# v1o/flyimg

Measured on AMD Instinct MI355X. Metric: input Mpix/s resize+smartcrop at 1/2/4/8 MI355X; % of HBM roofline, higher is better.
Workload: dtype u8

## Files before the change

### flyimg_amd/csrc/fi_batch.cpp

```cpp
#include "fi_runtime.h"

using namespace fi;

static int launch_batch(fi_ctx *c, const Exec &E, const BatchPlan &Bp, const Packed &K, uint8_t *ab, uint8_t *wb,
                        Slot &S) {
  S.tail = c->sc_stream;
  S.ap_lo = S.ap_hi = 0;
  const int32_t *ai = (const int32_t *)c->heap_i.p;
  const float *af = (const float *)c->heap_f.p;
  const double *ad = (const double *)c->heap_d.p;
  const ScParamsDev PD = to_dev(E.params);
  auto desc_p = [&](const Launch &L) { return ab + L.desc_off; };
  auto pre_p = [&](const Launch &L) { return (const int32_t *)(ab + L.prefix_off); };
  Timer tb(c, "batch", 0, c->stream, c->sc_stream);
  {
    Timer t(c, "resize", Bp.resize_bytes);
    if (K.L0.tiles)
      hipLaunchKernelGGL(k_rs_copy, dim3(K.L0.tiles), dim3(256), 0, c->stream, (const ResizeDesc *)desc_p(K.L0),
                         pre_p(K.L0), K.L0.n);
    const bool fork = c->vr_fork && c->rs2_stream && Bp.vrl.size() >= 2;
    if (fork) {
      if (!c->rs_fork) HIP_TRY(hipEventCreateWithFlags(&c->rs_fork, hipEventDisableTiming));
      if (!c->rs_join) HIP_TRY(hipEventCreateWithFlags(&c->rs_join, hipEventDisableTiming));
      HIP_TRY(hipEventRecord(c->rs_fork, c->stream));
// ... 331 lines not shown
    if (rc != FI_OK && first == FI_OK) first = rc;
  }
  if (first != FI_OK) return first;
  return FI_OK;
}
static int wait_slot(fi_ctx *c, int slot) {
  int first = FI_OK;
  while (c->slots[slot].busy && !c->inflight.empty()) {
    const int rc = finalize_front(c);
    if (rc != FI_OK && first == FI_OK) first = rc;
  }
  return first;
}

extern "C" {

int fi_debug_host_plan(const fi_image *imgs, int32_t n, int32_t iters, double *ms) {
  static fi_ctx *c = nullptr;
  static std::vector<uint8_t> last_blob;
  static size_t last_work = 0;
  static double last[7] = {0, 0, 0, 0, 0, 0, 0};
  if (!imgs && n == 0) {
    if (c && getenv("FI_PLAN_PROF"))
      for (const auto &kv : c->stats) fprintf(stderr, "%s %.1f ms (%lld)\n", kv.first.c_str(), kv.second.ms, (long long)kv.second.launches);
    delete c;
    c = nullptr;
    std::vector<uint8_t>().swap(last_blob);
    return FI_OK;
  }
  if (!imgs && n == 1) {
    if (c) c->stats.clear();
    return FI_OK;
  }
  if (!imgs && n == 2) {
    if (!ms) return set_err(FI_EINVAL, "ms is NULL");
    ms[0] = ms[1] = ms[2] = 0;
    if (c) {
      ms[0] = (double)c->stats["plan_path_vr"].launches;
      ms[1] = (double)c->stats["plan_vertical_first"].launches;
      ms[2] = (double)c->stats["plan_vr_launches"].launches;
    }
    return FI_OK;
  }
  if (!imgs && n == 3) {
    if (!ms) return set_err(FI_EINVAL, "ms is NULL");
    uint64_t h = 1469598103934665603ull;
    for (uint8_t x : last_blob) h = (h ^ x) * 1099511628211ull;
    for (int k = 0; k < 8; k++) h = (h ^ (((uint64_t)last_work >> (8 * k)) & 255)) * 1099511628211ull;
    last[0] = (double)(uint32_t)h;
    last[1] = (double)(uint32_t)(h >> 32);
    for (int k = 0; k < 7; k++) ms[k] = last[k];
    return FI_OK;
  }
  if (!imgs || n <= 0 || iters <= 0 || !ms) return set_err(FI_EINVAL, "bad arguments");
  if (!c) {
    c = new fi_ctx();
    c->host_only = true;
    c->timing = true;
    if (const char *e = getenv("FI_VR_RS")) c->vr_rs = e[0] == '1';
  }
  std::vector<fi_image> v(imgs, imgs + n);
  uint8_t *wb = reinterpret_cast<uint8_t *>((uintptr_t)1 << 40);
  int rc = FI_OK;
  for (int it = 0; it < iters && rc == FI_OK; it++) {
    const double t0 = now_ms();
    Exec E;
    E.c = c;
    fi_smartcrop_default_params(&E.params);
    rc = heap_prepare(c, E);
    if (rc) break;
    BatchPlan Bp;
    PlanTimes T;
    Packed K;
    const double vr0 = c->stats["host_plan_vr"].ms;
    plan_batch(c, E, Bp, v.data(), n, T);
    place_batch(c, E, Bp, K, wb, T);
    int nvr = 0;
    for (const BatchPlan::VrLaunch &V : Bp.vrl) nvr += V.images;
    c->stats["plan_path_vr"].launches += nvr;
    c->stats["plan_vertical_first"].launches += (int64_t)Bp.vdescs.size() - nvr;
    c->stats["plan_vr_launches"].launches += (int64_t)Bp.vrl.size();
    last_blob.swap(E.blob.b);
    last[2] = (double)last_blob.size();
    last[3] = (double)Bp.vtiles.size();
    last[4] = (double)Bp.vrtiles.size();
    last[5] = (double)Bp.htiles.size();
    last[6] = (double)Bp.sitems.size();
    last_work = E.work.size;
    if (!heap_fits(c, E)) heap_reset(c);
    else {
      c->heap_i.used = (size_t)E.bi + (E.ai.size() + 15) / 16 * 16;
      c->heap_f.used = (size_t)E.bf + (E.af.size() + 15) / 16 * 16;
      c->heap_d.used = (size_t)E.bd + (E.ad.size() + 15) / 16 * 16;
    }
    ms[0] += T.images - t0;
    ms[1] += T.sc - T.images;
    ms[2] += T.workspace - T.sc;
    ms[3] += T.vm - T.workspace;
    ms[4] += c->stats["host_plan_vr"].ms - vr0;
    ms[5] += T.hv - T.vm;
    ms[6] += T.blob - T.hv;
  }
  return rc;
}

int fi_process_batch_device(fi_ctx *c, fi_image *imgs, int32_t n) {
// ... 154 lines not shown
```

### flyimg_amd/csrc/fi_internal.h

```cpp
#pragma once
#include <hip/hip_runtime.h>
#include <stdint.h>

#include "../../include/flyimg_hip.h"

namespace fi {

constexpr int kMaxChannels = 3;

struct DevAxis {
  int32_t n;
  int32_t start;
  int32_t count;
  int32_t woff;
  int32_t maxtaps;
  int32_t src_lo;
  int32_t src_hi;
  int32_t touched;
  int32_t wbase;
  int32_t wd;
};

struct ResizeDesc {
  const uint8_t *src;
// ... 53 lines not shown
  int32_t ybox_first, hrows;
  int32_t hb, hk, ksh;
  int32_t vb, vk, ksv;
  int32_t hkT;
  int32_t prep;
  int32_t hm;
  int32_t hm_rows, hm_ks, hm_pitch, hm_nb;
  int32_t hmB, hmC, hmS0;
  int32_t vq;
  int32_t fz;
  int32_t fd;
  int32_t vqA, vqC, vqK0;
  int32_t cx;
  int32_t cx_kv, cx_tp;
  int32_t cxA, cxK0;
  int32_t cx_pad;
  uint8_t *tbuf;
  uint8_t *red;
  uint8_t *hbuf;
  uint8_t *pre;
  uint32_t *maps;
  int32_t crop0, ncrops;
  int32_t score0;
  double prescale;
  double T[3];
  int32_t result;
  int32_t exact_all;
  int32_t sg0, ngrp;
  int32_t sg_lds, sg_pad;
};

constexpr int kPrepRows = 16;
constexpr int kVqRows = 14;
constexpr int kPrepMaxLds = 64 * 1024;
constexpr int kHxRb = 8;
constexpr int kFzMaxLds = 80 * 1024;
__host__ __device__ inline uint32_t sc_spread3(uint32_t x) {
  x = (x | (x << 8)) & 0x0000F00Fu;
  x = (x | (x << 4)) & 0x000C30C3u;
  return (x | (x << 2)) & 0x00249249u;
}
__host__ __device__ inline uint32_t sc_colour_key(uint32_t r, uint32_t g, uint32_t b) {
  return (sc_spread3(r) << 2) | (sc_spread3(g) << 1) | sc_spread3(b);
}
constexpr int kFdSlots = 3;
constexpr int kFdCWaves = 14;
constexpr int kFdMaxLds = 160 * 1024;
__host__ __device__ inline int fd_rp(int W) { return (W * 3 + 15) & ~15; }
__host__ __device__ inline int fd_slot_bytes(int W) { return (16 * fd_rp(W) + 1023) & ~1023; }
__host__ __device__ inline int fd_ring_off(int W, int PP) {
  const int tail = 3 * PP - fd_rp(W);
  return kFdSlots * fd_slot_bytes(W) + (tail > 0 ? (tail + 15) & ~15 : 0);
}
__host__ __device__ inline int fd_tab_off(int W, int PP, int aw) {
  const int apitch = (aw * 3 + 15) & ~15, lpitch = (aw + 3) & ~3;
  return fd_ring_off(W, PP) + 80 * apitch + 16 * apitch + 16 * lpitch;
}
__host__ __device__ inline int fd_lds(int W, int PP, int aw, int ah) {
  return fd_tab_off(W, PP, aw) + (ah + kVqRows - 1) / kVqRows * 3072 + 4 * ah;
}
constexpr int kScoreLdsMaps = 112 * 1024;
constexpr int kScoreMaxCrops = 1024;
constexpr int kSgSlots = 3;
constexpr int kSgDigits = 5;
constexpr int kSgPlanes = 7;
constexpr int kSgMax = 2;
constexpr int kSgMaxKs = 2;
constexpr int kSgMaxCrops = kSgMax * 16 * kSgSlots;
constexpr int kScore3Lds = 160 * 1024 - 4608;
__host__ __device__ inline int sg_pitch(int aw) { return (aw + 7) & ~7; }
struct ScGroup {
  int32_t bfrag;
  int32_t nrows, ks, ybase;
  int32_t nm, nslot, q, step;
  int32_t x0[16];
  int32_t S[kSgDigits];
  int32_t pad[3];
};

#ifndef FI_MFMA_I8_MAP
#define FI_MFMA_I8_MAP 1
#endif
__host__ __device__ inline int mfma_i8_k(int l, int j) {
#if FI_MFMA_I8_MAP == 1
  return 16 * (l >> 4) + j;
#else
  return j < 8 ? 8 * (l >> 4) + j : 32 + 8 * (l >> 4) + (j - 8);
#endif
}
struct MStrip {
  int32_t x0, x1, b0, nbytes;
  int32_t c_lo, ncols, pitch, nocb, ks;
  int32_t lut_px0, lut_n;
  int32_t frag, s0, lut;
  int32_t vpitch;
  int32_t frag2;
};
constexpr int kHmMaxLds = 64 * 1024;

struct VDesc {
  const uint8_t *src;
  int64_t src_stride;
  uint8_t *dst;
  int64_t dst_stride;
  int32_t ew, eh, rot, gray;
  int32_t rows, nrows, row0, rstep;
  int32_t plo, pn, pblk, plast;
  int32_t pmeta;
  int32_t frag;
// ... 169 lines not shown
```

### flyimg_amd/csrc/fi_sc_plan.cpp

```cpp
#include "fi_runtime.h"

using namespace fi;

ScParamsDev fi::to_dev(const fi_smartcrop_params &p) {
  ScParamsDev d{};
  d.detail_weight = p.detail_weight;
  d.edge_radius = p.edge_radius;
  d.edge_weight = p.edge_weight;
  d.outside_importance = p.outside_importance;
  d.saturation_bias = p.saturation_bias;
  d.saturation_brightness_max = p.saturation_brightness_max;
  d.saturation_brightness_min = p.saturation_brightness_min;
  d.saturation_threshold = p.saturation_threshold;
  d.saturation_weight = p.saturation_weight;
  d.skin_bias = p.skin_bias;
  d.skin_brightness_max = p.skin_brightness_max;
  d.skin_brightness_min = p.skin_brightness_min;
  for (int i = 0; i < 3; i++) d.skin_color[i] = p.skin_color[i];
  d.skin_threshold = p.skin_threshold;
  d.skin_weight = p.skin_weight;
  d.rule_of_thirds = p.rule_of_thirds;
  return d;
}
static uint64_t params_hash(const fi_smartcrop_params &p) {
// ... 367 lines not shown
    } else if ((int64_t)d.aw * d.ah * 4 <= kScoreLdsMaps) {
      sl.push_back(d);
      X->sl_px = std::max(X->sl_px, d.aw * d.ah);
    } else {
      sg.push_back(d);
    }
  }
  X->red = add_launch(B, SL.descs, sred, [](const ScDesc &d) { return d.rh; });
  X->hp = add_launch(B, SL.descs, shp, [](const ScDesc &d) { return d.hrows; });
  X->vp = add_launch(B, SL.descs, svp, [](const ScDesc &d) { return d.ah; });
  X->maps = add_launch(B, SL.descs, smaps, [](const ScDesc &d) { return d.ah; });
  X->hm_off = B.addv(hm);
  X->nhm = (int)hm.size();
  X->vq_off = B.addv(vq);
  X->vm_off = B.addv(vm);
  X->nvm = (int)vm.size();
  X->nvq = (int)vq.size();
  X->fz_off = B.addv(fz);
  X->nfz = (int)fz.size();
  X->fd_off = B.addv(fd);
  X->nfd = (int)fd.size();
  X->cx_off = B.addv(cx);
  X->ncx = (int)cx.size();
  for (int v = 0; v < 4; v++) {
    const int ks = v / 2 + 1, nch = (v & 1) ? 3 : 1;
    std::vector<int32_t> ht, vt;
    for (size_t k = 0; k < cx.size(); k++) {
      const ScDesc &d = cx[k];
      if (d.C != nch) continue;
      if (d.hm_ks == ks)
        for (int r = 0; r < d.cx_tp / 16 - 1; r += kHxRb)
          for (int b = 0; b < d.hm_nb; b += 4) {
            ht.push_back((int32_t)k);
            ht.push_back(b);
            ht.push_back(r);
          }
      if (d.cx_kv == ks)
        for (int ch = 0; ch < (d.ah + kVqRows - 1) / kVqRows; ch++) {
          vt.push_back((int32_t)k);
          vt.push_back(ch);
        }
    }
    while (vt.size() % 8) {
      vt.push_back(-1);
      vt.push_back(0);
    }
    X->hxt_off[v] = B.addv(ht);
    X->hx_tiles[v] = (int)(ht.size() / 3);
    X->vxt_off[v] = B.addv(vt);
    X->vx_tiles[v] = (int)(vt.size() / 2);
  }
  c->stats["sc_path_cx"].launches += X->ncx;
  c->stats["sc_path_fd"].launches += X->nfd;
  c->stats["sc_path_fz"].launches += X->nfz;
  X->sl_off = B.addv(sl);
  X->nsl = (int)sl.size();
  X->sg_off = B.addv(sg);
  X->nsg = (int)sg.size();
  X->s3_off = B.addv(s3);
  X->ns3 = (int)s3.size();
  c->stats["sc_score_mfma"].launches += X->ns3;
  c->stats["sc_score_valu"].launches += X->nsl + X->nsg;
  X->groups_off = B.addv(SL.groups);
  X->crops_off = B.addv(SL.crops);
}
int fi::enqueue_sc(fi_ctx *c, hipStream_t st, uint8_t *ab, const ScLaunches &X, const int32_t *ai,
                      const double *ad, CropScore *scores, ScResult *results, const ScParamsDev &PD) {
  auto desc = [&](const Launch &L) { return (const ScDesc *)(ab + L.desc_off); };
  auto pre = [&](const Launch &L) { return (const int32_t *)(ab + L.prefix_off); };
  const uint16_t *skinsat = nullptr;
  if (X.nfz > 0 || X.nfd > 0 || X.ncx > 0) {
    const std::string key(reinterpret_cast<const char *>(&PD), offsetof(ScParamsDev, pad));
    if (!c->skinsat.p || c->skinsat_key != key) {
      const int rc = ensure(c, &c->skinsat, (size_t)2 << 24);
      if (rc != FI_OK) return rc;
      if (c->ap_pending && st == c->stream && order_after_apply(c) != FI_OK) return FI_EDEVICE;
      launch_sc_skinsat(st, (uint16_t *)c->skinsat.p, PD);
      c->skinsat_key = key;
    }
    skinsat = (const uint16_t *)c->skinsat.p;
  }
  {
    Timer t(c, "sc_prep", 0, st, st);
    if (X.red.tiles)
      hipLaunchKernelGGL(k_sc_reduce, dim3(X.red.tiles), dim3(256), 0, st, desc(X.red), pre(X.red), X.red.n);
    if (launch_sc_h(st, (const ScDesc *)(ab + X.hm_off), X.nhm, X.hm_chunks, X.hm_lds, ai) != 0 ||
        launch_sc_vq(st, (const ScDesc *)(ab + X.vq_off), X.nvq, X.vq_chunks, X.vq_lds, ai, PD) != 0 ||
        launch_sc_v(st, (const ScDesc *)(ab + X.vm_off), X.nvm, X.v_chunks, X.v_lds, ai, PD) != 0 ||
        launch_sc_fz(st, (const ScDesc *)(ab + X.fz_off), X.nfz, X.fz_lds, ai, PD, skinsat) != 0 ||
        launch_sc_fd(st, (const ScDesc *)(ab + X.fd_off), X.nfd, X.fd_lds, ai, PD, skinsat) != 0)
      return set_err(FI_EDEVICE, "smartcrop prescale launch rejected (LDS %d/%d/%d/%d)", X.hm_lds, X.vq_lds,
                     X.fz_lds, X.fd_lds);
    for (int v = 0; v < 4; v++) {
      const ScDesc *cd = (const ScDesc *)(ab + X.cx_off);
      if (launch_sc_hx(st, v / 2 + 1, (v & 1) ? 3 : 1, cd, (const int32_t *)(ab + X.hxt_off[v]), X.hx_tiles[v],
                       ai) != 0)
        return set_err(FI_EDEVICE, "k_sc_hx launch rejected");
    }
    for (int v = 0; v < 4; v++) {
      const ScDesc *cd = (const ScDesc *)(ab + X.cx_off);
      if (launch_sc_vx(st, v / 2 + 1, (v & 1) ? 3 : 1, cd, (const int32_t *)(ab + X.vxt_off[v]), X.vx_tiles[v],
                       ai, PD, skinsat) != 0)
        return set_err(FI_EDEVICE, "k_sc_vx launch rejected");
    }
    if (X.hp.tiles)
      hipLaunchKernelGGL(k_sc_hpass, dim3(X.hp.tiles), dim3(256), 0, st, desc(X.hp), pre(X.hp), X.hp.n, ai);
// ... 263 lines not shown
```

### flyimg_amd/csrc/fi_smartcrop.hip

```cpp
#include <hip/hip_runtime.h>
#include <stdint.h>

#include "fi_internal.h"
#include "fi_sc_device.h"

namespace fi {

constexpr int kPrepThreads = 256;


typedef int32_t i32x4 __attribute__((ext_vector_type(4)));
typedef int32_t i32x2 __attribute__((ext_vector_type(2)));

__global__ __launch_bounds__(kPrepThreads) void k_sc_hmfma(const ScDesc *__restrict__ descs,
                                                           const int32_t *__restrict__ ai) {
  extern __shared__ __attribute__((aligned(16))) uint8_t lds8[];
  const ScDesc &D = descs[blockIdx.x];
  const int R = D.hm_rows, P = D.hm_pitch, KS = D.hm_ks, nb = D.hm_nb;
  const int r0 = blockIdx.y * R;
  if (r0 >= D.hrows) return;
  const int tid = threadIdx.x, lane = tid & 63, wave = tid >> 6;
  const bool reduced = D.fx > 1 || D.fy > 1;
  const uint8_t *src = reduced ? D.red : D.img;
  const int64_t sstride = reduced ? (int64_t)D.rw * 3 : D.stride;
// ... 571 lines not shown
#pragma unroll
      for (int u = 0; u < kG; u++) {
        if (x_n >= aw) {
          x_n -= aw;
          yr_n++;
        }
        yrs[u] = yr_n;
        xs[u] = x_n;
        yr_n += stepy;
        x_n += stepx;
      }
      if (LUT) {
#pragma unroll
        for (int u = 0; u < kG; u++) {
          const int it = base + u * kFzThreads;
          sv[u] = 0;
          if (it < nit) {
            const uint8_t *qq = prer + (y0 + yrs[u] - pa) * apitch + 3 * xs[u];
            sv[u] = skinsat[sc_colour_key(qq[0], qq[1], qq[2])];
          }
        }
      }
#pragma unroll
      for (int u = 0; u < kG; u++) {
        const int it = base + u * kFzThreads;
        if (it >= nit) break;
        const int yr = yrs[u], x = xs[u], y = y0 + yr, m = y - pa;
        const uint8_t *lrow = lum + m * lpitch;
        const uint32_t L = lrow[x];
        uint32_t E = L;
        if (aw >= 3 && ah >= 3 && x > 0 && y > 0 && x < aw - 1 && y < ah - 1) {
          const int v = 4 * (int)L - (int)lrow[x - lpitch] - (int)lrow[x + lpitch] - (int)lrow[x - 1] - (int)lrow[x + 1] + 1;
          E = (uint32_t)(v <= 0 ? 0 : v >= 255 ? 255 : v);
        }
        uint32_t st;
        if (LUT) {
          st = (sv[u] & 255u) | ((sv[u] >> 8) << 16);
        } else {
          const uint8_t *qq = prer + m * apitch + 3 * x;
          st = sc_skin_sat(qq[0], qq[1], qq[2], L, P);
        }
        D.maps[(int64_t)y * aw + x] = st | (E << 8);
      }
    }
  }
}

constexpr int kFdThreads = 1024;
constexpr int kFdC = kFdCWaves * 64;
#ifndef FI_FD_ABL
#define FI_FD_ABL 0
#endif
constexpr int kFdAbl = FI_FD_ABL;
#ifndef FI_FD_LUT
#define FI_FD_LUT 0
#endif
constexpr bool kFdLut = FI_FD_LUT;
__device__ __forceinline__ void fd_dma16(uint32_t m0, const uint8_t *sbase, uint32_t voff) {
  unsigned keep;
  const uint64_t sb = (uint64_t)(uintptr_t)sbase;
  sbase = reinterpret_cast<const uint8_t *>((uintptr_t)(
      ((uint64_t)(uint32_t)__builtin_amdgcn_readfirstlane((int)(uint32_t)(sb >> 32)) << 32) |
      (uint32_t)__builtin_amdgcn_readfirstlane((int)(uint32_t)sb)));
  m0 = (uint32_t)__builtin_amdgcn_readfirstlane((int)m0);
  asm volatile(
      "s_mov_b32 %0, m0\n\t"
      "s_mov_b32 m0, %3\n\t"
      "s_nop 0\n\t"
      "global_load_lds_dwordx4 %1, %2\n\t"
      "s_mov_b32 m0, %0"
      : "=&s"(keep)
      : "v"(voff), "s"(sbase), "s"(m0)
      : "memory");
}
__device__ __forceinline__ void fd_wait_vm(int n) {
  switch (n) {
    case 0: asm volatile("s_waitcnt vmcnt(0)" ::: "memory"); break;
    case 1: asm volatile("s_waitcnt vmcnt(1)" ::: "memory"); break;
    case 2: asm volatile("s_waitcnt vmcnt(2)" ::: "memory"); break;
    case 3: asm volatile("s_waitcnt vmcnt(3)" ::: "memory"); break;
    case 4: asm volatile("s_waitcnt vmcnt(4)" ::: "memory"); break;
    case 5: asm volatile("s_waitcnt vmcnt(5)" ::: "memory"); break;
    case 6: asm volatile("s_waitcnt vmcnt(6)" ::: "memory"); break;
    case 7: asm volatile("s_waitcnt vmcnt(7)" ::: "memory"); break;
    case 8: asm volatile("s_waitcnt vmcnt(8)" ::: "memory"); break;
    case 9: asm volatile("s_waitcnt vmcnt(9)" ::: "memory"); break;
    case 10: asm volatile("s_waitcnt vmcnt(10)" ::: "memory"); break;
    case 11: asm volatile("s_waitcnt vmcnt(11)" ::: "memory"); break;
    case 12: asm volatile("s_waitcnt vmcnt(12)" ::: "memory"); break;
    case 13: asm volatile("s_waitcnt vmcnt(13)" ::: "memory"); break;
    case 14: asm volatile("s_waitcnt vmcnt(14)" ::: "memory"); break;
    default: asm volatile("s_waitcnt vmcnt(15)" ::: "memory"); break;
  }
}
__device__ __forceinline__ uint32_t fd_ch(int c, uint32_t a0, uint32_t a1, uint32_t a2) {
  const uint32_t s1 = c == 0 ? 0x00060300u : c == 1 ? 0x00070401u : 0x00000502u;
  const uint32_t s2 = c == 0 ? 0x05020100u : c == 1 ? 0x06020100u : 0x07040100u;
  return __builtin_amdgcn_perm(a2, __builtin_amdgcn_perm(a1, a0, s1), s2) ^ 0x80808080u;
}

__device__ __forceinline__ void fd_barrier() { asm volatile("s_waitcnt lgkmcnt(0)\n\ts_barrier" ::: "memory"); }

__global__ __launch_bounds__(kFdThreads) void k_sc_fd(const ScDesc *__restrict__ descs,
                                                      const int32_t *__restrict__ ai, const ScParamsDev P,
                                                      const uint16_t *__restrict__ skinsat) {
  extern __shared__ __attribute__((aligned(16))) uint8_t lds8[];
  const ScDesc &D = descs[blockIdx.x];
  const int tid = threadIdx.x, lane = tid & 63, wave = tid >> 6;
  const bool loader = wave >= kFdCWaves;
  const int aw = D.aw, ah = D.ah, hrows = D.hrows, yoff = D.ybox_first;
  const int apitch = (aw * 3 + 15) & ~15, lpitch = (aw + 3) & ~3;
  const int PP = D.hm_pitch, KS = D.hm_ks, nb = D.hm_nb;
  const int RP = fd_rp(D.W), slotB = fd_slot_bytes(D.W);
  const int64_t sstride = D.stride;
  uint8_t *raw = lds8;
  uint8_t *ring = lds8 + fd_ring_off(D.W, PP);
  uint8_t *prer = ring + kFzRing * apitch, *lum = prer + 16 * apitch;
  uint8_t *abuf = lds8 + fd_tab_off(D.W, PP, aw);
  const int chunks = (ah + kVqRows - 1) / kVqRows;
  int32_t *cbuf = reinterpret_cast<int32_t *>(abuf + chunks * 3072);
  const int nblk = (min(ai[D.vqK0 + chunks - 1] + 64, hrows) + 15) >> 4;
  const int ninstr = slotB >> 10, lw = wave - kFdCWaves;
  const int cnt = (ninstr - lw + 1) >> 1;
  const int rpc = RP >> 4;
  const float rcp_rpc = 1.0f / (float)rpc;
  const uint32_t raw_m0 = (uint32_t)(uintptr_t)(const __attribute__((address_space(3))) uint8_t *)raw;
  const uint32_t ab_m0 = (uint32_t)(uintptr_t)(const __attribute__((address_space(3))) uint8_t *)abuf;
  auto issue = [&](int blk) {
    if (blk >= nblk || (kFdAbl & 1)) return;
    const int r0 = blk << 4;
    const uint8_t *sb = D.img + (int64_t)(r0 + yoff) * sstride;
    const int last = hrows - 1 - r0;
#pragma unroll 1
    for (int i = lw; i < ninstr; i += 2) {
      const int j = 64 * i + lane;
      int row = fz_div(j, rpc, rcp_rpc);
      const int col = j - row * rpc;
      row = min(row, min(15, last));
      fd_dma16(raw_m0 + (uint32_t)((blk % kFdSlots) * slotB + 1024 * i), sb,
               (uint32_t)(row * sstride + 16 * col));
    }
  };
  const int32_t *hmS0 = ai + D.hmS0, *hmC = ai + D.hmC;
  const i32x4 *hmB = reinterpret_cast<const i32x4 *>(ai + D.hmB);
  const int k0l = mfma_i8_k(lane, 0), k8l = mfma_i8_k(lane, 8);
  auto load_b = [&](int b, i32x4 (&Bf)[2][3], int &s0, int32_t &cx) {
    s0 = hmS0[b];
#pragma unroll
    for (int t = 0; t < 2; t++)
#pragma unroll
      for (int q = 0; q < 3; q++) Bf[t][q] = t < KS ? hmB[((b * KS + t) * 3 + q) * 64 + lane] : i32x4{0, 0, 0, 0};
    const int x = 16 * b + (lane & 15);
    cx = x < aw ? hmC[x] : 0;
  };
  i32x4 Bh[2][3];
  int s0h = 0;
  int32_t cxh = 0;
  if (!loader && wave < nb) load_b(wave, Bh, s0h, cxh);
  auto hpass_block = [&](int r0, const uint8_t *slot, int b, const i32x4 (&Bf)[2][3], int s0, int32_t cx) {
    const int x = 16 * b + (lane & 15);
    i32x4 acc[3][3];
#pragma unroll
    for (int c = 0; c < 3; c++)
#pragma unroll
      for (int q = 0; q < 3; q++) acc[c][q] = i32x4{0, 0, 0, 0};
#pragma unroll
    for (int t = 0; t < 2; t++) {
      if (t < KS) {
        const uint8_t *rp = slot + (lane & 15) * RP + 3 * (s0 + 64 * t);
        const i32x2 *p0 = reinterpret_cast<const i32x2 *>(rp + 3 * k0l);
        const i32x2 *p1 = reinterpret_cast<const i32x2 *>(rp + 3 * k8l);
        const i32x2 u0 = p0[0], u1 = p0[1], u2 = p0[2], v0 = p1[0], v1 = p1[1], v2 = p1[2];
#pragma unroll
        for (int c = 0; c < 3; c++) {
          const i32x4 a = {(int32_t)fd_ch(c, u0.x, u0.y, u1.x), (int32_t)fd_ch(c, u1.y, u2.x, u2.y),
                           (int32_t)fd_ch(c, v0.x, v0.y, v1.x), (int32_t)fd_ch(c, v1.y, v2.x, v2.y)};
#pragma unroll
          for (int q = 0; q < 3; q++) acc[c][q] = __builtin_amdgcn_mfma_i32_16x16x64_i8(a, Bf[t][q], acc[c][q], 0, 0, 0);
        }
      }
    }
#pragma unroll
    for (int i = 0; i < 4; i++) {
      const int row = r0 + 4 * (lane >> 4) + i;
      if (x < aw && row < hrows) {
        uint8_t *dst = ring + (row % kFzRing) * apitch + 3 * x;
#pragma unroll
        for (int c = 0; c < 3; c++) {
          const uint32_t v = (uint32_t)acc[c][0][i] + ((uint32_t)acc[c][1][i] << 8) + ((uint32_t)acc[c][2][i] << 16) +
                             (uint32_t)cx;
          dst[c] = (uint8_t)(pil_clip8((int32_t)v) ^ 0x80u);
        }
      }
    }
  };
  auto hpass = [&](int r0, const uint8_t *slot) {
    if (wave < nb) hpass_block(r0, slot, wave, Bh, s0h, cxh);
  };
  const int rA = 16 * (lane >> 4) + ((lane & 15) >> 1);
  const int nq = apitch >> 4, nbytes = 3 * aw;
  const int stepy = kFdC / aw, stepx = kFdC - stepy * aw;
  const int lm0 = tid / aw, lx0 = tid - lm0 * aw;
  const ScFast F = sc_fast_params(P);
  const int ng4 = (aw + 3) >> 2;
  const float rcp_ng4 = 1.0f / (float)ng4;
  if (loader) {
    const uint8_t *afrag = reinterpret_cast<const uint8_t *>(ai + D.vqA);
#pragma unroll 1
    for (int k = lw; k < 3 * chunks; k += 2) fd_dma16(ab_m0 + 1024 * k, afrag, (uint32_t)(1024 * k + 16 * lane));
    issue(0);
    issue(1);
    fd_wait_vm(1 < nblk ? cnt : 0);
  } else {
#pragma unroll 1
    for (int i = tid; i < ah; i += kFdC) cbuf[i] = ai[D.vqC + i];
  }
  fd_barrier();
  int blk = 0;
#pragma unroll 1
  for (int c = 0; c < chunks; c++) {
    const int k0 = ai[D.vqK0 + c];
    const int need = min(k0 + 64, hrows);
    bool phased = false;
#pragma unroll 1
    while (16 * blk < need) {
      if (loader) {
        issue(blk + 2);
        fd_wait_vm(blk + 2 < nblk ? cnt : 0);
      } else if (!(kFdAbl & 2)) {
        hpass(16 * blk, raw + (blk % kFdSlots) * slotB);
      }
      fd_barrier();
      blk++;
      phased = true;
    }
    if (!phased) fd_barrier();
    const int y0 = kVqRows * c, y1 = min(y0 + kVqRows, ah), pa = max(0, y0 - 1), pe = min(ah, pa + 16);
    if (!loader) {
      const i32x4 *af = reinterpret_cast<const i32x4 *>(abuf + c * 3072);
      const i32x4 A0 = af[lane], A1 = af[64 + lane], A2 = af[128 + lane];
      int32_t cy[4];
#pragma unroll
      for (int i = 0; i < 4; i++) cy[i] = cbuf[min(pa + 4 * (lane >> 4) + i, ah - 1)];
      const uint8_t *pA = ring + ((k0 + rA) % kFzRing) * apitch + 8 * (lane & 1);
      const uint8_t *pB = ring + ((k0 + rA + 8) % kFzRing) * apitch + 8 * (lane & 1);
#pragma unroll 1
      for (int t = wave; t < ((kFdAbl & 4) ? 0 : nq); t += kFdCWaves) {
        const i32x2 lo = __builtin_amdgcn_ds_read_tr8_b64_v2i32((l_i32x2q *)(pA + 16 * t));
        const i32x2 hi = __builtin_amdgcn_ds_read_tr8_b64_v2i32((l_i32x2q *)(pB + 16 * t));
        const i32x4 B = {lo.x, lo.y, hi.x, hi.y};
        const i32x4 d2 = __builtin_amdgcn_mfma_i32_16x16x64_i8(A2, B, i32x4{0, 0, 0, 0}, 0, 0, 0);
        const i32x4 d1 = __builtin_amdgcn_mfma_i32_16x16x64_i8(A1, B, d2 << 8, 0, 0, 0);
        const i32x4 d0 = __builtin_amdgcn_mfma_i32_16x16x64_i8(A0, B, i32x4{0, 0, 0, 0}, 0, 0, 0);
        const int col = 16 * t + (lane & 15);
#pragma unroll
        for (int i = 0; i < 4; i++) {
          const int m = 4 * (lane >> 4) + i;
          const int32_t sv = (int32_t)((uint32_t)d0[i] + ((uint32_t)d1[i] << 8) + (uint32_t)cy[i]);
          if (col < nbytes && pa + m < pe) prer[m * apitch + col] = pil_clip8(sv);
        }
      }
    }
    fd_barrier();
    const int nit = (y1 - y0) * aw;
    int yr_n = lm0, x_n = lx0;
    uint32_t sv[kFzGather];
    auto walk = [&](int (&yrs)[kFzGather], int (&xs)[kFzGather]) {
#pragma unroll
      for (int u = 0; u < kFzGather; u++) {
        if (x_n >= aw) {
          x_n -= aw;
          yr_n++;
        }
        yrs[u] = yr_n;
        xs[u] = x_n;
        yr_n += stepy;
        x_n += stepx;
      }
    };
    auto gather = [&](int base) {
      int yrs[kFzGather], xs[kFzGather];
      walk(yrs, xs);
#pragma unroll
      for (int u = 0; u < kFzGather; u++) {
        const int it = base + u * kFdC;
        sv[u] = 0;
        if (it < nit) {
          const uint8_t *qq = prer + (y0 + yrs[u] - pa) * apitch + 3 * xs[u];
          sv[u] = (kFdAbl & 32) ? qq[0] * 0x101u : skinsat[sc_colour_key(qq[0], qq[1], qq[2])];
        }
      }
    };
    const int nr = pe - pa;
    if (!loader) {
      if (kFdLut && !(kFdAbl & 16)) gather(tid);
#pragma unroll 1
      for (int it = tid; it < ((kFdAbl & 8) ? 0 : nr * ng4); it += kFdC) {
        const int m = fz_div(it, ng4, rcp_ng4), g = it - m * ng4;
        const uint32_t *q = reinterpret_cast<const uint32_t *>(prer + m * apitch + 12 * g);
        const uint32_t a0 = q[0], a1 = q[1], a2 = q[2];
        const uint32_t R = fd_ch(0, a0, a1, a2) ^ 0x80808080u, G = fd_ch(1, a0, a1, a2) ^ 0x80808080u,
                       B = fd_ch(2, a0, a1, a2) ^ 0x80808080u;
        uint32_t l4 = 0;
#pragma unroll
        for (int j = 0; j < 4; j++)
          l4 |= sc_luma((R >> (8 * j)) & 255u, (G >> (8 * j)) & 255u, (B >> (8 * j)) & 255u) << (8 * j);
        *reinterpret_cast<uint32_t *>(lum + m * lpitch + 4 * g) = l4;
        const int y = pa + m;
        if (D.pre && y >= y0 && y < y1) {
#pragma unroll
          for (int j = 0; j < 4; j++) {
            const int x = 4 * g + j;
            if (x < aw) {
              uint8_t *o = D.pre + ((int64_t)y * aw + x) * 3;
              o[0] = (uint8_t)(R >> (8 * j));
              o[1] = (uint8_t)(G >> (8 * j));
              o[2] = (uint8_t)(B >> (8 * j));
            }
          }
        }
      }
    }
    fd_barrier();
    if (!loader && !kFdLut) {
      int yr_w = lm0, x_w = lx0;
#pragma unroll 1
      for (int base = tid; base < ((kFdAbl & 16) ? 0 : nit); base += kFzGather * kFdC) {
        uint32_t stv[kFzGather];
        int yrs[kFzGather], xs[kFzGather];
#pragma unroll
        for (int u = 0; u < kFzGather; u++) {
          if (x_w >= aw) {
            x_w -= aw;
            yr_w++;
          }
          yrs[u] = yr_w;
          xs[u] = x_w;
          yr_w += stepy;
          x_w += stepx;
          stv[u] = 0;
          if (base + u * kFdC < nit) {
            const int m = y0 + yrs[u] - pa;
            const uint8_t *qq = prer + m * apitch + 3 * xs[u];
            const uint32_t r = qq[0], g = qq[1], b = qq[2];
            if (!sc_skin_sat_est(F, r, g, b, lum[m * lpitch + xs[u]], stv[u])) {
              const uint32_t t = skinsat[sc_colour_key(r, g, b)];
              stv[u] = (t & 255u) | ((t >> 8) << 16);
            }
          }
        }
#pragma unroll
        for (int u = 0; u < kFzGather; u++) {
          const int it = base + u * kFdC;
          if (it >= nit) break;
          const int yr = yrs[u], x = xs[u], y = y0 + yr, m = y - pa;
          const uint8_t *lrow = lum + m * lpitch;
          const uint32_t L = lrow[x];
          uint32_t E = L;
          if (aw >= 3 && ah >= 3 && x > 0 && y > 0 && x < aw - 1 && y < ah - 1) {
            const int v = 4 * (int)L - (int)lrow[x - lpitch] - (int)lrow[x + lpitch] - (int)lrow[x - 1] - (int)lrow[x + 1] + 1;
            E = (uint32_t)(v <= 0 ? 0 : v >= 255 ? 255 : v);
          }
          if (!(kFdAbl & 64)) D.maps[(int64_t)y * aw + x] = stv[u] | (E << 8);
        }
      }
    }
    if (!loader && kFdLut) {
      yr_n = lm0;
      x_n = lx0;
#pragma unroll 1
      for (int base = tid; base < ((kFdAbl & 16) ? 0 : nit); base += kFzGather * kFdC) {
        if (base != tid) {
          const int ys = yr_n, xs0 = x_n;
          gather(base);
          yr_n = ys;
          x_n = xs0;
        }
        int yrs[kFzGather], xs[kFzGather];
        walk(yrs, xs);
#pragma unroll
        for (int u = 0; u < kFzGather; u++) {
          const int it = base + u * kFdC;
          if (it >= nit) break;
          const int yr = yrs[u], x = xs[u], y = y0 + yr, m = y - pa;
          const uint8_t *lrow = lum + m * lpitch;
          const uint32_t L = lrow[x];
          uint32_t E = L;
          if (aw >= 3 && ah >= 3 && x > 0 && y > 0 && x < aw - 1 && y < ah - 1) {
            const int v = 4 * (int)L - (int)lrow[x - lpitch] - (int)lrow[x + lpitch] - (int)lrow[x - 1] - (int)lrow[x + 1] + 1;
            E = (uint32_t)(v <= 0 ? 0 : v >= 255 ? 255 : v);
          }
          if (!(kFdAbl & 64)) D.maps[(int64_t)y * aw + x] = ((sv[u] & 255u) | ((sv[u] >> 8) << 16)) | (E << 8);
        }
      }
    }
  }
  if (loader) fd_wait_vm(0);
}

template <int KS, int NCH>
__global__ __launch_bounds__(256, KS == 2 && NCH == 3 ? 4 : 8) void k_sc_hx(const ScDesc *__restrict__ descs,
                                                                          const int32_t *__restrict__ tiles,
                                                                          const int32_t *__restrict__ ai) {
  typedef uint32_t u32x4a __attribute__((ext_vector_type(4), aligned(4)));
  const int wave = threadIdx.x >> 6, lane = threadIdx.x & 63;
  const int di = tiles[3 * blockIdx.x];
  if (di < 0) return;
  const ScDesc &D = descs[di];
  const int b = tiles[3 * blockIdx.x + 1] + wave, rb0 = tiles[3 * blockIdx.x + 2];
  if (b >= D.hm_nb) return;
  const int g = lane >> 4, r = lane & 15;
  const int aw = D.aw, hrows = D.hrows, yoff = D.ybox_first, tp = D.cx_tp;
  const int rp = NCH == 3 ? fd_rp(D.W) : (D.W + 15) & ~15;
  const int s0 = ai[D.hmS0 + b];
  const i32x4 *hmB = reinterpret_cast<const i32x4 *>(ai + D.hmB) + (size_t)b * KS * 3 * 64 + lane;
  constexpr bool kKeepB = !(KS == 2 && NCH == 3);
  i32x4 Bf[kKeepB ? KS : 1][3];
  if (kKeepB)
#pragma unroll
    for (int t = 0; t < KS; t++)
#pragma unroll
      for (int q = 0; q < 3; q++) Bf[kKeepB ? t : 0][q] = hmB[(t * 3 + q) * 64];
  auto bfrag = [&](int t, int q) {
    const i32x4 *hb = hmB;
    if (!kKeepB) asm volatile("" : "+v"(hb));
    return kKeepB ? Bf[kKeepB ? t : 0][q] : hb[(t * 3 + q) * 64];
  };
  const int x = 16 * b + r;
  const int32_t cxp = x < aw ? ai[D.hmC + x] - (1 << 29) : 0;
  constexpr int NQ = NCH == 3 ? 3 : 1;
  const int64_t sstride = D.stride;
  const int nrbt = tp >> 4;
  uint8_t *tcol = D.tbuf + (int64_t)b * NCH * nrbt * 256 + 16 * r + 4 * g;
  auto load = [&](int rb, u32x4a (&q)[KS][NQ]) {
    const int hr = min(16 * rb + r, hrows - 1);
    const uint8_t *row = D.img + (int64_t)(hr + yoff) * sstride;
#pragma unroll
    for (int t = 0; t < KS; t++)
#pragma unroll
      for (int i = 0; i < NQ; i++) {
        const int off = (NCH == 3 ? 3 : 1) * (s0 + 64 * t + 16 * g) + 16 * i;
        u32x4a v = *reinterpret_cast<const u32x4a *>(row + min(off, rp - 16));
        if (off > rp - 16) v = off == rp - 8 ? u32x4a{v.z, v.w, 0u, 0u} : u32x4a{0u, 0u, 0u, 0u};
        q[t][i] = v;
      }
// ... 917 lines not shown
```

Measured before the change: 950,500.

## Restructure fused smartcrop fd kernel to planar ring and register-resident vertical pass outputs

Changes the LDS ring layout in the fused fd smartcrop kernel from interleaved RGB rows to planar per-channel rows padded to 16 columns. The horizontal pass now splits per-block per-channel work items across waves and writes packed 4-byte words. The vertical pass keeps its RGB results in registers and computes luma, skin/saturation and the Laplacian edge directly using shuffles and a small double-buffered luma tile, removing the separate luma and gather passes and one barrier. It also adds a stats query for fd LDS usage. The risk is that the vertical pass now only runs on waves with index below nb, so wide images may leave columns unprocessed, and correctness depends on the new LDS size formula.

Measured after the change: 957,800 (median of 4 runs). Within noise of the previous version (+0.8%).

```diff
diff --git a/flyimg_amd/csrc/fi_batch.cpp b/flyimg_amd/csrc/fi_batch.cpp
--- a/flyimg_amd/csrc/fi_batch.cpp
+++ b/flyimg_amd/csrc/fi_batch.cpp
@@ -407,6 +407,17 @@
     for (int k = 0; k < 7; k++) ms[k] = last[k];
     return FI_OK;
   }
+  if (!imgs && n == 4) {
+    if (!ms) return set_err(FI_EINVAL, "ms is NULL");
+    ms[0] = ms[1] = ms[2] = 0;
+    ms[3] = (double)kFdMaxLds;
+    if (c) {
+      ms[0] = (double)c->stats["sc_path_fd"].launches;
+      ms[1] = (double)c->stats["sc_path_fz"].launches;
+      ms[2] = (double)c->stats["sc_fd_lds_max"].launches;
+    }
+    return FI_OK;
+  }
   if (!imgs || n <= 0 || iters <= 0 || !ms) return set_err(FI_EINVAL, "bad arguments");
   if (!c) {
     c = new fi_ctx();
diff --git a/flyimg_amd/csrc/fi_internal.h b/flyimg_amd/csrc/fi_internal.h
--- a/flyimg_amd/csrc/fi_internal.h
+++ b/flyimg_amd/csrc/fi_internal.h
@@ -129,9 +129,9 @@
   const int tail = 3 * PP - fd_rp(W);
   return kFdSlots * fd_slot_bytes(W) + (tail > 0 ? (tail + 15) & ~15 : 0);
 }
+__host__ __device__ inline int fd_xp(int aw) { return (aw + 15) & ~15; }
 __host__ __device__ inline int fd_tab_off(int W, int PP, int aw) {
-  const int apitch = (aw * 3 + 15) & ~15, lpitch = (aw + 3) & ~3;
-  return fd_ring_off(W, PP) + 80 * apitch + 16 * apitch + 16 * lpitch;
+  return fd_ring_off(W, PP) + 80 * 3 * fd_xp(aw) + 2 * 16 * fd_xp(aw);
 }
 __host__ __device__ inline int fd_lds(int W, int PP, int aw, int ah) {
   return fd_tab_off(W, PP, aw) + (ah + kVqRows - 1) / kVqRows * 3072 + 4 * ah;
diff --git a/flyimg_amd/csrc/fi_sc_plan.cpp b/flyimg_amd/csrc/fi_sc_plan.cpp
--- a/flyimg_amd/csrc/fi_sc_plan.cpp
+++ b/flyimg_amd/csrc/fi_sc_plan.cpp
@@ -443,6 +443,10 @@
   }
   c->stats["sc_path_cx"].launches += X->ncx;
   c->stats["sc_path_fd"].launches += X->nfd;
+  {
+    int64_t &m = c->stats["sc_fd_lds_max"].launches;
+    m = std::max<int64_t>(m, X->fd_lds);
+  }
   c->stats["sc_path_fz"].launches += X->nfz;
   X->sl_off = B.addv(sl);
   X->nsl = (int)sl.size();
diff --git a/flyimg_amd/csrc/fi_smartcrop.hip b/flyimg_amd/csrc/fi_smartcrop.hip
--- a/flyimg_amd/csrc/fi_smartcrop.hip
+++ b/flyimg_amd/csrc/fi_smartcrop.hip
@@ -647,10 +647,6 @@
 #define FI_FD_ABL 0
 #endif
 constexpr int kFdAbl = FI_FD_ABL;
-#ifndef FI_FD_LUT
-#define FI_FD_LUT 0
-#endif
-constexpr bool kFdLut = FI_FD_LUT;
 __device__ __forceinline__ void fd_dma16(uint32_t m0, const uint8_t *sbase, uint32_t voff) {
   unsigned keep;
   const uint64_t sb = (uint64_t)(uintptr_t)sbase;
@@ -693,6 +689,7 @@
   const uint32_t s2 = c == 0 ? 0x05020100u : c == 1 ? 0x06020100u : 0x07040100u;
   return __builtin_amdgcn_perm(a2, __builtin_amdgcn_perm(a1, a0, s1), s2) ^ 0x80808080u;
 }
+__device__ __forceinline__ uint32_t fd_byte(uint32_t v, int i) { return (v >> (8 * i)) & 255u; }
 
 __device__ __forceinline__ void fd_barrier() { asm volatile("s_waitcnt lgkmcnt(0)\n\ts_barrier" ::: "memory"); }
 
@@ -704,13 +701,15 @@
   const int tid = threadIdx.x, lane = tid & 63, wave = tid >> 6;
   const bool loader = wave >= kFdCWaves;
   const int aw = D.aw, ah = D.ah, hrows = D.hrows, yoff = D.ybox_first;
-  const int apitch = (aw * 3 + 15) & ~15, lpitch = (aw + 3) & ~3;
+  const int xp = fd_xp(aw), rpitch = 3 * xp;
   const int PP = D.hm_pitch, KS = D.hm_ks, nb = D.hm_nb;
   const int RP = fd_rp(D.W), slotB = fd_slot_bytes(D.W);
   const int64_t sstride = D.stride;
+  uint8_t *const pre = D.pre;
+  uint32_t *const maps = D.maps;
   uint8_t *raw = lds8;
   uint8_t *ring = lds8 + fd_ring_off(D.W, PP);
-  uint8_t *prer = ring + kFzRing * apitch, *lum = prer + 16 * apitch;
+  uint8_t *lumt = ring + kFzRing * rpitch;
   uint8_t *abuf = lds8 + fd_tab_off(D.W, PP, aw);
   const int chunks = (ah + kVqRows - 1) / kVqRows;
   int32_t *cbuf = reinterpret_cast<int32_t *>(abuf + chunks * 3072);
@@ -738,67 +737,91 @@
   };
   const int32_t *hmS0 = ai + D.hmS0, *hmC = ai + D.hmC;
   const i32x4 *hmB = reinterpret_cast<const i32x4 *>(ai + D.hmB);
-  const int k0l = mfma_i8_k(lane, 0), k8l = mfma_i8_k(lane, 8);
-  auto load_b = [&](int b, i32x4 (&Bf)[2][3], int &s0, int32_t &cx) {
-    s0 = hmS0[b];
-#pragma unroll
-    for (int t = 0; t < 2; t++)
-#pragma unroll
-      for (int q = 0; q < 3; q++) Bf[t][q] = t < KS ? hmB[((b * KS + t) * 3 + q) * 64 + lane] : i32x4{0, 0, 0, 0};
-    const int x = 16 * b + (lane & 15);
-    cx = x < aw ? hmC[x] : 0;
-  };
-  i32x4 Bh[2][3];
-  int s0h = 0;
-  int32_t cxh = 0;
-  if (!loader && wave < nb) load_b(wave, Bh, s0h, cxh);
-  auto hpass_block = [&](int r0, const uint8_t *slot, int b, const i32x4 (&Bf)[2][3], int s0, int32_t cx) {
-    const int x = 16 * b + (lane & 15);
-    i32x4 acc[3][3];
-#pragma unroll
-    for (int c = 0; c < 3; c++)
-#pragma unroll
-      for (int q = 0; q < 3; q++) acc[c][q] = i32x4{0, 0, 0, 0};
-#pragma unroll
-    for (int t = 0; t < 2; t++) {
-      if (t < KS) {
-        const uint8_t *rp = slot + (lane & 15) * RP + 3 * (s0 + 64 * t);
-        const i32x2 *p0 = reinterpret_cast<const i32x2 *>(rp + 3 * k0l);
-        const i32x2 *p1 = reinterpret_cast<const i32x2 *>(rp + 3 * k8l);
-        const i32x2 u0 = p0[0], u1 = p0[1], u2 = p0[2], v0 = p1[0], v1 = p1[1], v2 = p1[2];
-#pragma unroll
-        for (int c = 0; c < 3; c++) {
-          const i32x4 a = {(int32_t)fd_ch(c, u0.x, u0.y, u1.x), (int32_t)fd_ch(c, u1.y, u2.x, u2.y),
-                           (int32_t)fd_ch(c, v0.x, v0.y, v1.x), (int32_t)fd_ch(c, v1.y, v2.x, v2.y)};
-#pragma unroll
-          for (int q = 0; q < 3; q++) acc[c][q] = __builtin_amdgcn_mfma_i32_16x16x64_i8(a, Bf[t][q], acc[c][q], 0, 0, 0);
-        }
-      }
-    }
+  const int g = lane >> 4, n = lane & 15;
+  int it0 = 0, it1 = 0;
+  if (!loader && KS == 1) {
+    const int nitems = 3 * nb, s = wave & 3, j = wave >> 2;
+    const int sbase = nitems >> 2, srem = nitems & 3;
+    const int si0 = s * sbase + min(s, srem), sn = sbase + (s < srem ? 1 : 0);
+    const int nws = (kFdCWaves - s + 3) >> 2;
+    const int wbase = sn / nws, wrem = sn - wbase * nws;
+    it0 = si0 + j * wbase + min(j, wrem);
+    it1 = it0 + wbase + (j < wrem ? 1 : 0);
+  } else if (!loader && wave < nb) {
+    it0 = 3 * wave;
+    it1 = it0 + 3;
+  }
+  it0 = __builtin_amdgcn_readfirstlane(it0);
+  it1 = __builtin_amdgcn_readfirstlane(it1);
+  const int hb0 = it0 / 3;
+  i32x4 Fs[2][3];
+  int s0h[2] = {0, 0};
+  int32_t cxh[2][4];
+#pragma unroll
+  for (int h = 0; h < 2; h++) {
+    const int b = hb0 + h;
+    const bool have = it0 < it1 && 3 * b < it1;
+    const bool slot = KS == 1 ? have : it0 < it1;
+    const int f = KS == 1 ? b : 2 * hb0 + h;
+#pragma unroll
+    for (int q = 0; q < 3; q++) Fs[h][q] = slot ? hmB[(f * 3 + q) * 64 + lane] : i32x4{0, 0, 0, 0};
+    if (have) s0h[h] = hmS0[b];
 #pragma unroll
     for (int i = 0; i < 4; i++) {
-      const int row = r0 + 4 * (lane >> 4) + i;
-      if (x < aw && row < hrows) {
-        uint8_t *dst = ring + (row % kFzRing) * apitch + 3 * x;
-#pragma unroll
-        for (int c = 0; c < 3; c++) {
-          const uint32_t v = (uint32_t)acc[c][0][i] + ((uint32_t)acc[c][1][i] << 8) + ((uint32_t)acc[c][2][i] << 16) +
-                             (uint32_t)cx;
-          dst[c] = (uint8_t)(pil_clip8((int32_t)v) ^ 0x80u);
-        }
-      }
+      const int x = 16 * b + 4 * g + i;
+      cxh[h][i] = have && x < aw ? hmC[x] : 0;
+    }
+  }
+  auto hpass_block = [&](int r0, const uint8_t *slot, int b, int clo, int chi, const i32x4 (&F0)[3],
+                         const i32x4 (&F1)[3], int s0, const int32_t (&cx)[4]) {
+    const i32x2 *p = reinterpret_cast<const i32x2 *>(slot + n * RP + 3 * (s0 + 16 * g));
+    i32x2 u[6], v[6];
+#pragma unroll
+    for (int k = 0; k < 6; k++) u[k] = p[k];
+#pragma unroll
+    for (int k = 0; k < 6; k++) v[k] = i32x2{0, 0};
+    if (KS == 2)
+#pragma unroll
+      for (int k = 0; k < 6; k++) v[k] = p[24 + k];
+    uint8_t *dst = ring + (r0 % kFzRing + n) * rpitch + 16 * b + 4 * g;
+#pragma unroll 1
+    for (int c = clo; c < chi; c++) {
+      i32x4 acc0 = {cx[0], cx[1], cx[2], cx[3]}, acc1 = {0, 0, 0, 0}, acc2 = {0, 0, 0, 0};
+      const i32x4 px = {(int32_t)fd_ch(c, u[0].x, u[0].y, u[1].x), (int32_t)fd_ch(c, u[1].y, u[2].x, u[2].y),
+                        (int32_t)fd_ch(c, u[3].x, u[3].y, u[4].x), (int32_t)fd_ch(c, u[4].y, u[5].x, u[5].y)};
+      acc0 = __builtin_amdgcn_mfma_i32_16x16x64_i8(F0[0], px, acc0, 0, 0, 0);
+      acc1 = __builtin_amdgcn_mfma_i32_16x16x64_i8(F0[1], px, acc1, 0, 0, 0);
+      acc2 = __builtin_amdgcn_mfma_i32_16x16x64_i8(F0[2], px, acc2, 0, 0, 0);
+      if (KS == 2) {
+        const i32x4 py = {(int32_t)fd_ch(c, v[0].x, v[0].y, v[1].x), (int32_t)fd_ch(c, v[1].y, v[2].x, v[2].y),
+                          (int32_t)fd_ch(c, v[3].x, v[3].y, v[4].x), (int32_t)fd_ch(c, v[4].y, v[5].x, v[5].y)};
+        acc0 = __builtin_amdgcn_mfma_i32_16x16x64_i8(F1[0], py, acc0, 0, 0, 0);
+        acc1 = __builtin_amdgcn_mfma_i32_16x16x64_i8(F1[1], py, acc1, 0, 0, 0);
+        acc2 = __builtin_amdgcn_mfma_i32_16x16x64_i8(F1[2], py, acc2, 0, 0, 0);
+      }
+      uint32_t w = 0;
+#pragma unroll
+      for (int i = 0; i < 4; i++) {
+        const uint32_t a = (uint32_t)acc0[i] + ((uint32_t)acc1[i] << 8) + ((uint32_t)acc2[i] << 16);
+        w |= (uint32_t)pil_clip8((int32_t)a) << (8 * i);
+      }
+      if (r0 + n < hrows) *reinterpret_cast<uint32_t *>(dst + c * xp) = w ^ 0x80808080u;
     }
   };
   auto hpass = [&](int r0, const uint8_t *slot) {
-    if (wave < nb) hpass_block(r0, slot, wave, Bh, s0h, cxh);
+#pragma unroll
+    for (int h = 0; h < 2; h++) {
+      const int b = hb0 + h;
+      const int clo = max(it0, 3 * b) - 3 * b, chi = min(it1, 3 * b + 3) - 3 * b;
+      if (clo < chi) hpass_block(r0, slot, b, clo, chi, Fs[h], Fs[1], s0h[h], cxh[h]);
+    }
   };
-  const int rA = 16 * (lane >> 4) + ((lane & 15) >> 1);
-  const int nq = apitch >> 4, nbytes = 3 * aw;
-  const int stepy = kFdC / aw, stepx = kFdC - stepy * aw;
-  const int lm0 = tid / aw, lx0 = tid - lm0 * aw;
+  const bool vact = !loader && wave < nb;
+  const int x = 16 * wave + n;
+  const int rA = 16 * g + (n >> 1);
+  const int tro = 8 * (lane & 1) + 16 * wave;
   const ScFast F = sc_fast_params(P);
-  const int ng4 = (aw + 3) >> 2;
-  const float rcp_ng4 = 1.0f / (float)ng4;
+  const bool edges = aw >= 3 && ah >= 3;
   if (loader) {
     const uint8_t *afrag = reinterpret_cast<const uint8_t *>(ai + D.vqA);
 #pragma unroll 1
@@ -816,7 +839,6 @@
   for (int c = 0; c < chunks; c++) {
     const int k0 = ai[D.vqK0 + c];
     const int need = min(k0 + 64, hrows);
-    bool phased = false;
 #pragma unroll 1
     while (16 * blk < need) {
       if (loader) {
@@ -827,165 +849,73 @@
       }
       fd_barrier();
       blk++;
-      phased = true;
-    }
-    if (!phased) fd_barrier();
-    const int y0 = kVqRows * c, y1 = min(y0 + kVqRows, ah), pa = max(0, y0 - 1), pe = min(ah, pa + 16);
-    if (!loader) {
-      const i32x4 *af = reinterpret_cast<const i32x4 *>(abuf + c * 3072);
-      const i32x4 A0 = af[lane], A1 = af[64 + lane], A2 = af[128 + lane];
-      int32_t cy[4];
-#pragma unroll
-      for (int i = 0; i < 4; i++) cy[i] = cbuf[min(pa + 4 * (lane >> 4) + i, ah - 1)];
-      const uint8_t *pA = ring + ((k0 + rA) % kFzRing) * apitch + 8 * (lane & 1);
-      const uint8_t *pB = ring + ((k0 + rA + 8) % kFzRing) * apitch + 8 * (lane & 1);
-#pragma unroll 1
-      for (int t = wave; t < ((kFdAbl & 4) ? 0 : nq); t += kFdCWaves) {
-        const i32x2 lo = __builtin_amdgcn_ds_read_tr8_b64_v2i32((l_i32x2q *)(pA + 16 * t));
-        const i32x2 hi = __builtin_amdgcn_ds_read_tr8_b64_v2i32((l_i32x2q *)(pB + 16 * t));
-        const i32x4 B = {lo.x, lo.y, hi.x, hi.y};
-        const i32x4 d2 = __builtin_amdgcn_mfma_i32_16x16x64_i8(A2, B, i32x4{0, 0, 0, 0}, 0, 0, 0);
-        const i32x4 d1 = __builtin_amdgcn_mfma_i32_16x16x64_i8(A1, B, d2 << 8, 0, 0, 0);
-        const i32x4 d0 = __builtin_amdgcn_mfma_i32_16x16x64_i8(A0, B, i32x4{0, 0, 0, 0}, 0, 0, 0);
-        const int col = 16 * t + (lane & 15);
-#pragma unroll
-        for (int i = 0; i < 4; i++) {
-          const int m = 4 * (lane >> 4) + i;
-          const int32_t sv = (int32_t)((uint32_t)d0[i] + ((uint32_t)d1[i] << 8) + (uint32_t)cy[i]);
-          if (col < nbytes && pa + m < pe) prer[m * apitch + col] = pil_clip8(sv);
-        }
-      }
+    }
+    const int y0 = kVqRows * c, y1 = min(y0 + kVqRows, ah), pa = max(0, y0 - 1);
+    uint8_t *lt = lumt + (c & 1) * 16 * xp;
+    uint32_t rgb[3] = {0, 0, 0}, L4 = 0;
+    if (vact) {
+      if (!(kFdAbl & 4)) {
+        const i32x4 *af = reinterpret_cast<const i32x4 *>(abuf + c * 3072);
+        const i32x4 A0 = af[lane], A1 = af[64 + lane], A2 = af[128 + lane];
+        int32_t cy[4];
+#pragma unroll
+        for (int i = 0; i < 4; i++) cy[i] = cbuf[min(pa + 4 * g + i, ah - 1)];
+        const uint8_t *pA = ring + ((k0 + rA) % kFzRing) * rpitch + tro;
+        const uint8_t *pB = ring + ((k0 + rA + 8) % kFzRing) * rpitch + tro;
+#pragma unroll
+        for (int ch = 0; ch < 3; ch++) {
+          const i32x2 lo = __builtin_amdgcn_ds_read_tr8_b64_v2i32((l_i32x2q *)(pA + ch * xp));
+          const i32x2 hi = __builtin_amdgcn_ds_read_tr8_b64_v2i32((l_i32x2q *)(pB + ch * xp));
+          const i32x4 B = {lo.x, lo.y, hi.x, hi.y};
+          const i32x4 d2 = __builtin_amdgcn_mfma_i32_16x16x64_i8(A2, B, i32x4{0, 0, 0, 0}, 0, 0, 0);
+          const i32x4 d1 = __builtin_amdgcn_mfma_i32_16x16x64_i8(A1, B, d2 << 8, 0, 0, 0);
+          const i32x4 d0 = __builtin_amdgcn_mfma_i32_16x16x64_i8(A0, B, i32x4{0, 0, 0, 0}, 0, 0, 0);
+          uint32_t w = 0;
+#pragma unroll
+          for (int i = 0; i < 4; i++) {
+            const int32_t sv = (int32_t)((uint32_t)d0[i] + ((uint32_t)d1[i] << 8) + (uint32_t)cy[i]);
+            w |= (uint32_t)pil_clip8(sv) << (8 * i);
+          }
+          rgb[ch] = w;
+        }
+      }
+#pragma unroll
+      for (int i = 0; i < 4; i++)
+        L4 |= sc_luma(fd_byte(rgb[0], i), fd_byte(rgb[1], i), fd_byte(rgb[2], i)) << (8 * i);
+      *reinterpret_cast<uint32_t *>(lt + 16 * x + 4 * g) = L4;
     }
     fd_barrier();
-    const int nit = (y1 - y0) * aw;
-    int yr_n = lm0, x_n = lx0;
-    uint32_t sv[kFzGather];
-    auto walk = [&](int (&yrs)[kFzGather], int (&xs)[kFzGather]) {
-#pragma unroll
-      for (int u = 0; u < kFzGather; u++) {
-        if (x_n >= aw) {
-          x_n -= aw;
-          yr_n++;
-        }
-        yrs[u] = yr_n;
-        xs[u] = x_n;
-        yr_n += stepy;
-        x_n += stepx;
-      }
-    };
-    auto gather = [&](int base) {
-      int yrs[kFzGather], xs[kFzGather];
-      walk(yrs, xs);
-#pragma unroll
-      for (int u = 0; u < kFzGather; u++) {
-        const int it = base + u * kFdC;
-        sv[u] = 0;
-        if (it < nit) {
-          const uint8_t *qq = prer + (y0 + yrs[u] - pa) * apitch + 3 * xs[u];
-          sv[u] = (kFdAbl & 32) ? qq[0] * 0x101u : skinsat[sc_colour_key(qq[0], qq[1], qq[2])];
-        }
-      }
-    };
-    const int nr = pe - pa;
-    if (!loader) {
-      if (kFdLut && !(kFdAbl & 16)) gather(tid);
-#pragma unroll 1
-      for (int it = tid; it < ((kFdAbl & 8) ? 0 : nr * ng4); it += kFdC) {
-        const int m = fz_div(it, ng4, rcp_ng4), g = it - m * ng4;
-        const uint32_t *q = reinterpret_cast<const uint32_t *>(prer + m * apitch + 12 * g);
-        const uint32_t a0 = q[0], a1 = q[1], a2 = q[2];
-        const uint32_t R = fd_ch(0, a0, a1, a2) ^ 0x80808080u, G = fd_ch(1, a0, a1, a2) ^ 0x80808080u,
-                       B = fd_ch(2, a0, a1, a2) ^ 0x80808080u;
-        uint32_t l4 = 0;
-#pragma unroll
-        for (int j = 0; j < 4; j++)
-          l4 |= sc_luma((R >> (8 * j)) & 255u, (G >> (8 * j)) & 255u, (B >> (8 * j)) & 255u) << (8 * j);
-        *reinterpret_cast<uint32_t *>(lum + m * lpitch + 4 * g) = l4;
-        const int y = pa + m;
-        if (D.pre && y >= y0 && y < y1) {
-#pragma unroll
-          for (int j = 0; j < 4; j++) {
-            const int x = 4 * g + j;
-            if (x < aw) {
-              uint8_t *o = D.pre + ((int64_t)y * aw + x) * 3;
-              o[0] = (uint8_t)(R >> (8 * j));
-              o[1] = (uint8_t)(G >> (8 * j));
-              o[2] = (uint8_t)(B >> (8 * j));
-            }
-          }
-        }
-      }
-    }
-    fd_barrier();
-    if (!loader && !kFdLut) {
-      int yr_w = lm0, x_w = lx0;
-#pragma unroll 1
-      for (int base = tid; base < ((kFdAbl & 16) ? 0 : nit); base += kFzGather * kFdC) {
-        uint32_t stv[kFzGather];
-        int yrs[kFzGather], xs[kFzGather];
-#pragma unroll
-        for (int u = 0; u < kFzGather; u++) {
-          if (x_w >= aw) {
-            x_w -= aw;
-            yr_w++;
-          }
-          yrs[u] = yr_w;
-          xs[u] = x_w;
-          yr_w += stepy;
-          x_w += stepx;
-          stv[u] = 0;
-          if (base + u * kFdC < nit) {
-            const int m = y0 + yrs[u] - pa;
-            const uint8_t *qq = prer + m * apitch + 3 * xs[u];
-            const uint32_t r = qq[0], g = qq[1], b = qq[2];
-            if (!sc_skin_sat_est(F, r, g, b, lum[m * lpitch + xs[u]], stv[u])) {
-              const uint32_t t = skinsat[sc_colour_key(r, g, b)];
-              stv[u] = (t & 255u) | ((t >> 8) << 16);
-            }
-          }
-        }
-#pragma unroll
-        for (int u = 0; u < kFzGather; u++) {
-          const int it = base + u * kFdC;
-          if (it >= nit) break;
-          const int yr = yrs[u], x = xs[u], y = y0 + yr, m = y - pa;
-          const uint8_t *lrow = lum + m * lpitch;
-          const uint32_t L = lrow[x];
-          uint32_t E = L;
-          if (aw >= 3 && ah >= 3 && x > 0 && y > 0 && x < aw - 1 && y < ah - 1) {
-            const int v = 4 * (int)L - (int)lrow[x - lpitch] - (int)lrow[x + lpitch] - (int)lrow[x - 1] - (int)lrow[x + 1] + 1;
-            E = (uint32_t)(v <= 0 ? 0 : v >= 255 ? 255 : v);
-          }
-          if (!(kFdAbl & 64)) D.maps[(int64_t)y * aw + x] = stv[u] | (E << 8);
-        }
-      }
-    }
-    if (!loader && kFdLut) {
-      yr_n = lm0;
-      x_n = lx0;
-#pragma unroll 1
-      for (int base = tid; base < ((kFdAbl & 16) ? 0 : nit); base += kFzGather * kFdC) {
-        if (base != tid) {
-          const int ys = yr_n, xs0 = x_n;
-          gather(base);
-          yr_n = ys;
-          x_n = xs0;
-        }
-        int yrs[kFzGather], xs[kFzGather];
-        walk(yrs, xs);
-#pragma unroll
-        for (int u = 0; u < kFzGather; u++) {
-          const int it = base + u * kFdC;
-          if (it >= nit) break;
-          const int yr = yrs[u], x = xs[u], y = y0 + yr, m = y - pa;
-          const uint8_t *lrow = lum + m * lpitch;
-          const uint32_t L = lrow[x];
-          uint32_t E = L;
-          if (aw >= 3 && ah >= 3 && x > 0 && y > 0 && x < aw - 1 && y < ah - 1) {
-            const int v = 4 * (int)L - (int)lrow[x - lpitch] - (int)lrow[x + lpitch] - (int)lrow[x - 1] - (int)lrow[x + 1] + 1;
-            E = (uint32_t)(v <= 0 ? 0 : v >= 255 ? 255 : v);
-          }
-          if (!(kFdAbl & 64)) D.maps[(int64_t)y * aw + x] = ((sv[u] & 255u) | ((sv[u] >> 8) << 16)) | (E << 8);
+    if (vact && !(kFdAbl & 16)) {
+      const uint32_t up = (uint32_t)__shfl((int)L4, lane - 16, 64), dn = (uint32_t)__shfl((int)L4, lane + 16, 64);
+      const uint32_t lf = *reinterpret_cast<const uint32_t *>(lt + 16 * max(x - 1, 0) + 4 * g);
+      const uint32_t rt = *reinterpret_cast<const uint32_t *>(lt + 16 * min(x + 1, xp - 1) + 4 * g);
+      uint32_t stv[4];
+#pragma unroll
+      for (int i = 0; i < 4; i++) {
+        const uint32_t rr = fd_byte(rgb[0], i), gg = fd_byte(rgb[1], i), bb = fd_byte(rgb[2], i);
+        if (!sc_skin_sat_est(F, rr, gg, bb, fd_byte(L4, i), stv[i])) {
+          const uint32_t t = (kFdAbl & 32) ? rr * 0x101u : skinsat[sc_colour_key(rr, gg, bb)];
+          stv[i] = (t & 255u) | ((t >> 8) << 16);
+        }
+      }
+#pragma unroll
+      for (int i = 0; i < 4; i++) {
+        const int y = pa + 4 * g + i;
+        if (x >= aw || y < y0 || y >= y1) continue;
+        const uint32_t L = fd_byte(L4, i);
+        uint32_t E = L;
+        if (edges && x > 0 && y > 0 && x < aw - 1 && y < ah - 1) {
+          const uint32_t u = i > 0 ? fd_byte(L4, i - 1) : fd_byte(up, 3);
+          const uint32_t d = i < 3 ? fd_byte(L4, i + 1) : fd_byte(dn, 0);
+          const int v = 4 * (int)L - (int)u - (int)d - (int)fd_byte(lf, i) - (int)fd_byte(rt, i) + 1;
+          E = (uint32_t)(v <= 0 ? 0 : v >= 255 ? 255 : v);
+        }
+        if (!(kFdAbl & 64)) maps[(int64_t)y * aw + x] = stv[i] | (E << 8);
+        if (pre) {
+          uint8_t *o = pre + ((int64_t)y * aw + x) * 3;
+          o[0] = (uint8_t)fd_byte(rgb[0], i);
+          o[1] = (uint8_t)fd_byte(rgb[1], i);
+          o[2] = (uint8_t)fd_byte(rgb[2], i);
         }
       }
     }
```
